# GATB/dsk

Measured on AMD Instinct MI355X. Metric: distinct k-mers counted/sec (whole node), k=31, higher is better.
Workload: dtype u64

## Files before the change

dsk_amd/csrc/dskgpu.hip:

```cpp
#include <algorithm>
#include <cstdio>
#include <cstring>
#include <cstdlib>
#include <cmath>
#include <string>
#include <vector>

#include <thread>
#include <system_error>
#include "engine.h"
#include "kernels.h"
#include "superkmer_recv.h"
#include "rawparse.h"

#include <rocprim/device/device_radix_sort.hpp>

#define DSKGPU_VERSION "dskgpu 0.1 (gfx950)"

namespace {

thread_local std::string g_create_err;

__global__ __launch_bounds__(1024) void k_place_probe(unsigned long long* __restrict__ out, unsigned long long n) {
    const unsigned long long per_block = n / gridDim.x, per_stream = per_block / 512;
// ... 115 lines not shown
    if ((reinterpret_cast<uintptr_t>(d_bytes) & 15) == 0)
        hipLaunchKernelGGL(k_encode<true>, dim3(grid), dim3(256), 0, ctx->stream, d_bytes, n, packed, inval, nwords);
    else
        hipLaunchKernelGGL(k_encode<false>, dim3(grid), dim3(256), 0, ctx->stream, d_bytes, n, packed, inval, nwords);
    CKL("k_encode");
    return DSKGPU_OK;
}

int run_scan(dskgpu_ctx* ctx, u32* a, const u32* d_len, u64 max_len) {
    const u64 nb = std::max<u64>(1, (max_len + SCAN_BLK - 1) / SCAN_BLK);
    CK(ctx->sums.ensure((nb + 1) * 4));
    hipLaunchKernelGGL(k_scan_reduce, dim3((unsigned)nb), dim3(SCAN_NT), 0, ctx->stream, a, d_len, ctx->sums.as<u32>());
    hipLaunchKernelGGL(k_scan_sums, dim3(1), dim3(1024), 0, ctx->stream, ctx->sums.as<u32>(), d_len, a);
    hipLaunchKernelGGL(k_scan_apply, dim3((unsigned)nb), dim3(SCAN_NT), 0, ctx->stream, a, d_len, ctx->sums.as<u32>());
    CKL("k_scan");
    return DSKGPU_OK;
}

int allow_big_lds(dskgpu_ctx* ctx, const void* fn, int bytes) {
    for (const void* f : ctx->big_lds_fns) if (f == fn) return DSKGPU_OK;
    CK(hipFuncSetAttribute(fn, hipFuncAttributeMaxDynamicSharedMemorySize, bytes));
    ctx->big_lds_fns.push_back(fn);
    return DSKGPU_OK;
}

namespace {

size_t scatter_lds(int W, u32 P, bool opt = false) { return (size_t)SC_NT * (16 / W) * 8 * W + (size_t)P * (opt ? 20 : 16) + 4 + 17 * 4 + 16 + (opt ? 8 + L0_MAX_PASSES * 8 : 0); }

template <int W, int SRC, int MODE>
int launch_hist_m(dskgpu_ctx* ctx, const typename KeyT<W>::T* keys, const ChunkDesc* descs, const u32* d_nch,
                  u64 max_chunks, u32* matrix, DigitSpec ds, u32 P) {
    const unsigned grid = (unsigned)std::max<u64>(1, std::min<u64>(max_chunks, (u64)ctx->num_cu));
    hipLaunchKernelGGL((k_hist<W, SRC, MODE>), dim3(grid), dim3(SC_NT), 0, ctx->stream, ctx->packed.as<u64>(),
                       ctx->inval.as<u32>(), keys, descs, d_nch, matrix, (int)ctx->cfg.kmer_size, ds, P);
    CKL("k_hist");
    return DSKGPU_OK;
}
template <int W, int SRC>
int launch_hist(dskgpu_ctx* ctx, const typename KeyT<W>::T* keys, const ChunkDesc* descs, const u32* d_nch,
                u64 max_chunks, u32* matrix, DigitSpec ds, u32 P) {
    const bool mp = ds.mode == 1 && ds.npass > 1;
    if (SRC == 0) return ds.mode == 0 ? launch_hist_m<W, 0, 0>(ctx, keys, descs, d_nch, max_chunks, matrix, ds, P)
                       : mp ? launch_hist_m<W, 0, 3>(ctx, keys, descs, d_nch, max_chunks, matrix, ds, P)
                            : launch_hist_m<W, 0, 1>(ctx, keys, descs, d_nch, max_chunks, matrix, ds, P);
    return ds.mode == 2 ? launch_hist_m<W, 1, 2>(ctx, keys, descs, d_nch, max_chunks, matrix, ds, P)
                   : mp ? launch_hist_m<W, 1, 3>(ctx, keys, descs, d_nch, max_chunks, matrix, ds, P)
                        : launch_hist_m<W, 1, 1>(ctx, keys, descs, d_nch, max_chunks, matrix, ds, P);
}

unsigned scatter_grid(const dskgpu_ctx* ctx, int W, u32 P, u64 max_chunks, bool opt = false) {
    const size_t lds = scatter_lds(W, P, opt);
    const u64 per_cu = std::max<u64>(1, std::min<u64>(2048 / SC_NT, (160 * 1024) / lds));
    return (unsigned)std::max<u64>(1, std::min<u64>(max_chunks, (u64)ctx->num_cu * per_cu));
}
template <int W, int SRC, int MODE, bool OPT = false, bool HEAVY = false>
int launch_scatter_m(dskgpu_ctx* ctx, const typename KeyT<W>::T* keys, const ChunkDesc* descs, const u32* d_nch,
                     u64 max_chunks, const u32* scanned, typename KeyT<W>::T* out, DigitSpec ds, u32 P, Opt1Spec o1 = Opt1Spec{nullptr, 0u, 0u, nullptr, nullptr, 0u, nullptr, nullptr, nullptr, 0u, nullptr, 0ull, {0ull, 0ull, 0ull, 0ull}, 0u}) {
    const size_t lds = scatter_lds(W, P, OPT && !o1.uslice);
    const unsigned grid = scatter_grid(ctx, W, P, max_chunks, OPT && !o1.uslice);
    { const int e = allow_big_lds(ctx, reinterpret_cast<const void*>(&k_scatter<W, SRC, MODE, OPT, HEAVY>)); if (e) return e; }
    hipLaunchKernelGGL((k_scatter<W, SRC, MODE, OPT, HEAVY>), dim3(grid), dim3(SC_NT), lds, ctx->stream, SRC == 2 ? ctx->rec_src : ctx->packed.as<u64>(),
                       SRC == 2 ? nullptr : ctx->inval.as<u32>(), keys, descs, d_nch, scanned, out, (int)ctx->cfg.kmer_size, ds, P, o1);
    CKL("k_scatter");
    return DSKGPU_OK;
}
template <int W, int MODE, bool OPT = false, bool SLICED = false>
int launch_scatter_al(dskgpu_ctx* ctx, const typename KeyT<W>::T* keys, const ChunkDesc* descs, const u32* d_nch,
                      u64 max_chunks, const u32* scanned, typename KeyT<W>::T* out, DigitSpec ds, u32 P, OptSpec os = OptSpec{0u, nullptr, nullptr, nullptr, 0u, 0u, 0ull, 0u, 0u, nullptr, nullptr, nullptr, nullptr, nullptr, nullptr}) {
    const size_t lds = ascatter_lds(W, P);
    const unsigned grid = (unsigned)std::max<u64>(1, std::min<u64>(max_chunks, (u64)ctx->num_cu));
    { const int e = allow_big_lds(ctx, reinterpret_cast<const void*>(&k_scatter_al<W, MODE, OPT, SLICED>)); if (e) return e; }
    hipLaunchKernelGGL((k_scatter_al<W, MODE, OPT, SLICED>), dim3(grid), dim3(SC_NT), lds, ctx->stream, keys, descs, d_nch, scanned, out, ds, P, os);
    CKL("k_scatter_al");
    return DSKGPU_OK;
}

template <int W, int SRC>
int launch_scatter(dskgpu_ctx* ctx, const typename KeyT<W>::T* keys, const ChunkDesc* descs, const u32* d_nch,
                   u64 max_chunks, const u32* scanned, typename KeyT<W>::T* out, DigitSpec ds, u32 P) {
    const bool mp = ds.mode == 1 && ds.npass > 1;
    if (SRC == 1 && ascatter_lds(W, P) <= 160 * 1024 && !ctx->tune.no_aligned)
        return ds.mode == 2 ? launch_scatter_al<W, 2>(ctx, keys, descs, d_nch, max_chunks, scanned, out, ds, P)
                       : mp ? launch_scatter_al<W, 3>(ctx, keys, descs, d_nch, max_chunks, scanned, out, ds, P)
                            : launch_scatter_al<W, 1>(ctx, keys, descs, d_nch, max_chunks, scanned, out, ds, P);
    if (SRC == 0) return ds.mode == 0 ? launch_scatter_m<W, 0, 0>(ctx, keys, descs, d_nch, max_chunks, scanned, out, ds, P)
                       : mp ? launch_scatter_m<W, 0, 3>(ctx, keys, descs, d_nch, max_chunks, scanned, out, ds, P)
                            : launch_scatter_m<W, 0, 1>(ctx, keys, descs, d_nch, max_chunks, scanned, out, ds, P);
    return ds.mode == 2 ? launch_scatter_m<W, 1, 2>(ctx, keys, descs, d_nch, max_chunks, scanned, out, ds, P)
                   : mp ? launch_scatter_m<W, 1, 3>(ctx, keys, descs, d_nch, max_chunks, scanned, out, ds, P)
                        : launch_scatter_m<W, 1, 1>(ctx, keys, descs, d_nch, max_chunks, scanned, out, ds, P);
}

inline void launch_count_impl(dskgpu_ctx* ctx, unsigned grid, u64* keys, u64* solid_keys, u32* solid_ab, u32* ovf, const CountParams& cp) {
    if (cp.cap && cp.cap <= CNT_V3_KEYS * CNT_NT) {
        hipLaunchKernelGGL((k_count1v3<CNT_NT, CNT_KPT, CNT_V3_KEYS>), dim3(grid), dim3(CNT_NT), 0, ctx->stream, keys, solid_keys, solid_ab,
                           ctx->nsolid.as<u32>(), ctx->ghist.as<u64>(), ctx->gstats.as<u64>(), ovf, cp, cp.subcnt);
        return;
    }
    if (cp.cap) hipLaunchKernelGGL(k_count1<true>, dim3(grid), dim3(CNT_NT), 0, ctx->stream, keys, solid_keys, ctx->fstart.as<u32>(), solid_ab,
                                   ctx->nsolid.as<u32>(), ctx->ghist.as<u64>(), ctx->gstats.as<u64>(), ovf, cp, cp.subcnt);
    else hipLaunchKernelGGL(k_count1<false>, dim3(grid), dim3(CNT_NT), 0, ctx->stream, keys, solid_keys, ctx->fstart.as<u32>(), solid_ab,
                            ctx->nsolid.as<u32>(), ctx->ghist.as<u64>(), ctx->gstats.as<u64>(), ovf, cp, (const u32*)ctx->fstart.as<u32>());
}
template <int W>
inline void launch_count_impl(dskgpu_ctx* ctx, unsigned grid, KN<W>* keys, KN<W>* solid_keys, u32* solid_ab, u32* ovf, const CountParams& cp) {
    if constexpr (W == 2) {
// ... 549 lines not shown
    ctx->mark("scatter1");
    return DSKGPU_OK;
}

template <int W>
int pass_scatter2(dskgpu_ctx* ctx, PassState<W>& ps) {
    const Plan& pl = ps.pl;
    int rc;
    ps.fkeys = ctx->bufA.as<typename KeyT<W>::T>();
    ps.scratch = &ctx->bufB;
    CK(ctx->fstart.ensure(((size_t)pl.F + 2) * 4));
    CK(ctx->nsolid.ensure(((size_t)pl.F + 2) * 4));
    if (pl.levels == 2 && ps.opt_cap) {
        CK(ctx->bufB.ensure((ps.nregions * ps.opt_cap + ATile<W>::KEYS + 16) * sizeof(typename KeyT<W>::T)));
        CK(ctx->descs2.ensure(((size_t)pl.P1 * 2 + 1) * sizeof(ChunkDesc)));
        CK(ctx->seg.ensure((size_t)pl.P1 * sizeof(SegInfo)));
        CK(ctx->mat2.ensure(((size_t)ps.nregions + 1) * 4));
        CK(ctx->chain_next.ensure(((size_t)ps.nregions + 1 + ps.max_ext + 1) * 4));
        if (ps.opt1) {
            ctx->h_descs2.resize(pl.P1);
            std::vector<u32> order(pl.P1);
            for (u32 sgm = 0; sgm < pl.P1; ++sgm) order[sgm] = sgm;
            double mean_work = 0.0; for (double w : ps.load) mean_work += w; mean_work = std::max(1.0, mean_work / pl.P1);
            auto wclass = [&](u32 a) { return (long long)(ps.load[a] / (0.05 * mean_work)); };
            std::stable_sort(order.begin(), order.end(), [&](u32 a, u32 b) { return wclass(a) > wclass(b); });
            for (u32 i = 0; i < pl.P1; ++i) {
                const u32 sgm = order[i];
                ChunkDesc d; d.begin = ctx->h_boff[sgm]; d.end = ctx->h_boff[sgm + 1]; d.flat_base = sgm * pl.P2; d.stride = 1;
                ctx->h_descs2[i] = d;
            }
            CK(hipMemcpyAsync(ctx->descs2.p, ctx->h_descs2.data(), (size_t)pl.P1 * sizeof(ChunkDesc), hipMemcpyHostToDevice, ctx->stream));
        } else {
            hipLaunchKernelGGL(k_plan, dim3(1), dim3(1024), 0, ctx->stream, ctx->mat1.as<u32>(), ps.nch1, pl.P1, 0x7FFFFFFFu, pl.P2,
                               ctx->seg.as<SegInfo>(), ctx->descs2.as<ChunkDesc>(), ps.sc + SC_NCH2, ps.sc + SC_MLEN2, 1u);
            CKL("k_plan");
        }
        ctx->mark("plan2");
        OptSpec os{ps.opt_cap, ctx->mat2.as<u32>(), ps.sc + SC_OVF2, ps.opt1 ? ps.o1.fill : nullptr, 0u, ps.grid1, (u64)ps.o1.area,
                   pl.F, ps.max_ext, ctx->chain_next.as<u32>(), ps.sc + SC_EXT, ctx->chain_next.as<u32>() + ps.nregions + 1, ps.sc + SC_NCHAINED,
                   ps.sc + SC_WORK2, nullptr};
        if (ctx->tune.verbose && ps.opt1) { CK(ctx->dbg.ensure((size_t)pl.P1 * 24)); os.dbg = ctx->dbg.as<unsigned long long>(); }
        if (ps.opt1) rc = launch_scatter_al<W, 2, true, true>(ctx, ctx->bufA.as<typename KeyT<W>::T>(), ctx->descs2.as<ChunkDesc>(), ps.sc + SC_NCH2, (u64)pl.P1 * 2, nullptr,
                                                              ctx->bufB.as<typename KeyT<W>::T>(), pl.d2, pl.P2, os);
        else rc = launch_scatter_al<W, 2, true, false>(ctx, ctx->bufA.as<typename KeyT<W>::T>(), ctx->descs2.as<ChunkDesc>(), ps.sc + SC_NCH2, (u64)pl.P1 * 2, nullptr,
                                                       ctx->bufB.as<typename KeyT<W>::T>(), pl.d2, pl.P2, os);
        if (rc) return rc;
        ctx->mark("scatter2");
        if (ctx->tune.verbose && ps.opt1) {
            std::vector<unsigned long long> t((size_t)pl.P1 * 3);
            CK(hipMemcpyAsync(t.data(), ctx->dbg.p, t.size() * 8, hipMemcpyDeviceToHost, ctx->stream));
            CK(hipStreamSynchronize(ctx->stream));
            unsigned long long t0 = ~0ull, t1 = 0; for (u32 i = 0; i < pl.P1; ++i) { t0 = std::min(t0, t[3 * i]); t1 = std::max(t1, t[3 * i + 1]); }
            fprintf(stderr, "[dskgpu] level 2: %u segments, %.3f ms first start -> last end\n", pl.P1, (t1 - t0) * 1e-5);
            for (u32 i = 0; i < pl.P1; ++i)
                if (i < 6 || i + 3 >= pl.P1 || t[3 * i + 1] + 20000 > t1)
                    fprintf(stderr, "[dskgpu]   desc %u (segment %u, load %.0f) block %llu: %.3f .. %.3f ms\n", i, (u32)(ctx->h_descs2[i].flat_base / pl.P2),
                            ps.load[ctx->h_descs2[i].flat_base / pl.P2], t[3 * i + 2], (t[3 * i] - t0) * 1e-5, (t[3 * i + 1] - t0) * 1e-5);
        }
        ps.fkeys = ctx->bufB.as<typename KeyT<W>::T>();
        ps.scratch = &ctx->bufA;
    } else if (pl.levels == 2) {
        const u64 max_chunks2 = ps.cap / CH2 + pl.P1 + 1;
        const u64 M2 = max_chunks2 * pl.P2;
        if (M2 >= 0xFFFFFFFFull) return fail(ctx, DSKGPU_E_ARG, "level-2 matrix too large");
        CK(ctx->descs2.ensure(max_chunks2 * sizeof(ChunkDesc)));
        CK(ctx->seg.ensure((size_t)pl.P1 * sizeof(SegInfo)));
        CK(ctx->mat2.ensure((M2 + 1) * 4));
        hipLaunchKernelGGL(k_plan, dim3(1), dim3(1024), 0, ctx->stream, ctx->mat1.as<u32>(), ps.nch1, pl.P1, CH2, pl.P2,
                           ctx->seg.as<SegInfo>(), ctx->descs2.as<ChunkDesc>(), ps.sc + SC_NCH2, ps.sc + SC_MLEN2, 0u);
        CKL("k_plan");
        ctx->mark("plan2");
        const ChunkDesc* dd2 = ctx->descs2.as<ChunkDesc>();
        if ((rc = launch_hist<W, 1>(ctx, ctx->bufA.as<typename KeyT<W>::T>(), dd2, ps.sc + SC_NCH2, max_chunks2, ctx->mat2.as<u32>(), pl.d2, pl.P2))) return rc;
        ctx->mark("hist2");
        if ((rc = run_scan(ctx, ctx->mat2.as<u32>(), ps.sc + SC_MLEN2, M2))) return rc;
        ctx->mark("scan2");
        if ((rc = launch_scatter<W, 1>(ctx, ctx->bufA.as<typename KeyT<W>::T>(), dd2, ps.sc + SC_NCH2, max_chunks2, ctx->mat2.as<u32>(), ctx->bufB.as<typename KeyT<W>::T>(), pl.d2, pl.P2))) return rc;
        ctx->mark("scatter2");
        ps.fkeys = ctx->bufB.as<typename KeyT<W>::T>();
        ps.scratch = &ctx->bufA;
        hipLaunchKernelGGL(k_final_offsets, dim3((pl.F + 256) / 256), dim3(256), 0, ctx->stream, ctx->mat2.as<u32>(),
                           ctx->seg.as<SegInfo>(), pl.P2, 0u, ps.sc + SC_MLEN2, ctx->fstart.as<u32>(), pl.F);
    } else {
        hipLaunchKernelGGL(k_final_offsets, dim3((pl.F + 256) / 256), dim3(256), 0, ctx->stream, ctx->mat1.as<u32>(),
                           (const SegInfo*)nullptr, pl.P1, ps.nch1, ps.sc + SC_MLEN1, ctx->fstart.as<u32>(), pl.F);
    }
    CKL("k_final_offsets");
    ctx->mark("offsets");
    return DSKGPU_OK;
}

template <int W>
int count_and_sizes(dskgpu_ctx* ctx, PassState<W>& ps, const CountParams& cp) {
    typedef typename KeyT<W>::T Key;
    const Plan& pl = ps.pl;
    const unsigned cgrid = (unsigned)std::min<u64>(pl.F, (u64)ctx->num_cu * 2);
    launch_count<W>(ctx, cgrid, ps.fkeys, ps.solid_keys, ps.solid_ab, ps.sc + SC_OVERFLOW, cp);
    CKL("k_count");
    if constexpr (W <= 2) {
        if (ps.opt_cap && ps.max_ext) {
            auto kern = [] { if constexpr (W == 1) return k_count_chained; else return k_count_chained_mw<2>; }();
            hipLaunchKernelGGL(kern, dim3((unsigned)std::min<u64>(ps.max_ext, (u64)ctx->num_cu * 2)), dim3(CNT_NT), 0, ctx->stream, ps.fkeys, ps.solid_keys, ps.solid_ab,
                               ctx->nsolid.as<u32>(), ctx->ghist.as<u64>(), ctx->gstats.as<u64>(), ps.sc + SC_OVERFLOW, cp, (const u32*)cp.subcnt,
                               (const u32*)ctx->chain_next.as<u32>(), (const u32*)(ctx->chain_next.as<u32>() + ps.nregions + 1), (const u32*)(ps.sc + SC_NCHAINED), ps.max_ext);
            CKL(W == 1 ? "k_count_chained" : "k_count_chained_mw");
        }
        if (ps.nheavy) {
            const u32 slots = HV_KEYS;
            u64* hvb = ctx->hv_buf.as<u64>();
            hipLaunchKernelGGL(k_heavy_rows<W>, dim3((slots + 255) / 256), dim3(256), 0, ctx->stream, reinterpret_cast<const Key*>(hvb + HvLayout<W>::keys),
// ... 1227 lines not shown
```

dsk_amd/csrc/engine.h:

```cpp
#pragma once
#include <algorithm>
#include <cstring>
#include <string>
#include <vector>

#include "../../include/dskgpu.h"
#include "layouts.h"

hipError_t placed_malloc(void** out, size_t bytes);

struct DevBuf {
    void* p = nullptr;
    size_t cap = 0;
    hipError_t ensure(size_t bytes) {
        if (bytes <= cap) return hipSuccess;
        size_t want = ((p ? bytes + bytes / 16 : bytes) + 255) & ~size_t(255);
        if (p) { (void)hipFree(p); p = nullptr; cap = 0; }
        hipError_t e = placed_malloc(&p, want);
        if (e == hipSuccess) cap = want; else p = nullptr;
        return e;
    }
    int ensure_keep(size_t bytes, size_t keep, hipStream_t stream) {
        if (bytes <= cap) return 0;
        void* np = nullptr;
        size_t want = ((std::max(bytes, cap + cap / 2) + 255) & ~size_t(255));
        if (hipMalloc(&np, want) != hipSuccess) return -1;
        if (keep && p) {
            if (hipMemcpyAsync(np, p, keep, hipMemcpyDeviceToDevice, stream) != hipSuccess || hipStreamSynchronize(stream) != hipSuccess) { (void)hipFree(np); return -1; }
        }
        if (p) (void)hipFree(p);
        p = np; cap = want;
        return 0;
    }
    void release() { if (p) (void)hipFree(p); p = nullptr; cap = 0; }
    template <class T> T* as() const { return reinterpret_cast<T*>(p); }
};

enum Scalar { SC_NCH1 = 0, SC_MLEN1, SC_NCH2, SC_MLEN2, SC_OVERFLOW, SC_F, SC_SORTFLAG, SC_OVF2, SC_OVF1, SC_RSLEN, SC_RSWORK, SC_RSWORK2, SC_RSTIES, SC_EXT, SC_NCHAINED, SC_NCH_S, SC_MLEN_S, SC_WORK2, SC_COUNT = 24 };

struct Stage { const char* name; hipEvent_t ev; };

struct Tuning {
    bool no_opt1 = false, no_opt2 = false;
    bool no_aligned = false;
    u32 rs_heavy = 0;
    u32 rs_bbits = 0;
    u32 rs_block_rows = 0;
    bool sk_exact = false, no_recsrc = false;
    u32 opt_cap = 0;
    u64 opt_slice = 0;
    u64 sk_slice = 0, sk_minslice = 2000;
    u32 table_maxload = 0;
    long long max_ext = -1;
    bool no_sample = false;
    bool no_heavy = false;
    bool verbose = false;
    bool no_level0 = false; u32 l0_passes = 0;
    u64 rs_max_rows = 0;
    u32 ps_maxc = 0;
    bool sk_generic = false;
    bool l0_keys = false;
    u32 mp_pass_mkeys = 0;
    u64 rs_slab_rows = 0;
    bool unitig_stages = false;
    bool cc_plain = false, cc_stages = false;
    bool correct_staged = false;
    u32 pairs_reg_max = ~0u, pairs_grid = 0; bool pairs_no_skip = false;
    void read() {
        auto on =[](const char* n) { return getenv(n) != nullptr; };
        auto num = [](const char* n, u64 dflt) { const char* e = getenv(n); return e ? (u64)atoll(e) : dflt; };
        no_opt1 = on("DSKGPU_NO_OPT1"); no_opt2 = on("DSKGPU_NO_OPT2"); no_aligned = on("DSKGPU_NO_ALIGNED");
        sk_exact = on("DSKGPU_SK_EXACT");
        no_recsrc = on("DSKGPU_NO_RECSRC");
        opt_cap = (u32)num("DSKGPU_OPT_CAP", 0) & ~7u; opt_slice = num("DSKGPU_OPT_SLICE", 0) & ~7ull;
        sk_slice = num("DSKGPU_SK_SLICE", 0); sk_minslice = num("DSKGPU_SK_MINSLICE", 2000);
        table_maxload = (u32)num("DSKGPU_TABLE_MAXLOAD", 0);
        max_ext = getenv("DSKGPU_MAX_EXT") ? atoll(getenv("DSKGPU_MAX_EXT")) : -1;
        no_sample = on("DSKGPU_NO_SAMPLE"); no_heavy = on("DSKGPU_NO_HEAVY"); verbose = on("DSKGPU_VERBOSE"); no_level0 = on("DSKGPU_NO_LEVEL0"); l0_passes = (u32)num("DSKGPU_L0_PASSES", 0); mp_pass_mkeys = (u32)num("DSKGPU_MP_PASS_MKEYS", 0); rs_max_rows = num("DSKGPU_RS_MAX_ROWS", 0); l0_keys = on("DSKGPU_L0_KEYS"); sk_generic = on("DSKGPU_SK_GENERIC"); ps_maxc = (u32)num("DSKGPU_PS_MAXC", 0);
        rs_slab_rows = num("DSKGPU_RS_SLAB_ROWS", 0);
        unitig_stages = on("DSKGPU_UNITIG_STAGES");
        cc_plain = on("DSKGPU_CC_PLAIN"); cc_stages = on("DSKGPU_CC_STAGES");
        correct_staged = on("DSKGPU_CORRECT_STAGED");
        pairs_reg_max = (u32)num("DSKGPU_PAIRS_REG_MAX", pairs_reg_max); pairs_no_skip = on("DSKGPU_PAIRS_NO_SKIP"); pairs_grid = (u32)num("DSKGPU_PAIRS_GRID", 0);
        rs_block_rows = (u32)num("DSKGPU_RS_BLOCK_ROWS", 0); rs_bbits = (u32)num("DSKGPU_RS_BBITS", 0); rs_heavy = (u32)num("DSKGPU_RS_HEAVY", 0);
    }
};

struct SparseRows {
    int W = 0;
    const void* keys = nullptr; const u32 *ab = nullptr, *soff = nullptr, *fstart = nullptr; u32 cap = 0, F = 0;
    u64 n_sparse = 0; u32 n_tail = 0; RowsIn tail_w{}; const u32* tail_ab = nullptr;
    template <class S> S as(u32 qpc = 0) const { return S{static_cast<decltype(S::keys)>(keys), ab, soff, fstart, cap, F, qpc}; }
    Rows2C tail2() const { return Rows2C{tail_w.w[1], tail_w.w[0], tail_ab}; }
};

struct PartPasses {
    struct Pass { u64 row_base; u32 nparts, off_index; };
    std::vector<Pass> passes; DevBuf part_off, flag; u32 off_used = 0; bool ok = false; u64 row_base = 0;
    std::vector<u32> h_off;
};

struct RowSort {
    DevBuf fix_list;
    DevBuf g[4];
    DevBuf del, lens;
    std::vector<u64> h_del; std::vector<u32> h_lens, h_lin;
    DevBuf ovs;
    u32 flag = 0, listed = 0;
    u64* hist_pin = nullptr; size_t hist_pin_n = 0;
    bool part_mode = false; u32 n_parts = 0; u32* h_part_off = nullptr; size_t h_part_cap = 0; DevBuf part_off;
    std::vector<u64> h_part_off64;
    PartPasses mp;
    void release() {
        for (DevBuf* b : {&fix_list, &g[0], &g[1], &g[2], &g[3], &del, &lens, &ovs, &part_off, &mp.part_off, &mp.flag}) b->release();
        if (hist_pin) (void)hipHostFree(hist_pin);
        if (h_part_off) (void)hipHostFree(h_part_off);
        hist_pin = nullptr; h_part_off = nullptr;
    }
};

struct Query {
    DevBuf table, packed, inval, deg;
    u64 cap = 0;
    bool valid = false;
    void release() { table.release(); packed.release(); inval.release(); deg.release(); cap = 0; valid = false; }
    void invalidate() { valid = false; }
};

struct Components {
    DevBuf comp, first, cols;
    dskgpu_component_stats stats{};
    bool valid = false;
// ... 248 lines not shown
```

dsk_amd/csrc/kernels.h:

```cpp
#pragma once
#include "layouts.h"

#ifndef SC_NT
#define SC_NT 1024
#endif
template <int W> struct Tile {
    static constexpr int KPT = 16 / W;
    static constexpr int KEYS = SC_NT * KPT;
    static constexpr int WORDS = KEYS / 32;
};
#define MAX_BINS 2048


template <bool ALIGNED>
__global__ __launch_bounds__(256) void k_encode(const uint8_t* __restrict__ s, u64 n,
                                                u64* __restrict__ packed, u32* __restrict__ inval, u64 nwords) {
    const u64 stride = (u64)gridDim.x * blockDim.x;
    for (u64 w = (u64)blockIdx.x * blockDim.x + threadIdx.x; w < nwords; w += stride) {
        const u64 base = w * 32;
        u32 x[8];
        if (ALIGNED && base + 32 <= n) {
            const uint4 a = *reinterpret_cast<const uint4*>(s + base);
            const uint4 b = *reinterpret_cast<const uint4*>(s + base + 16);
            x[0] = a.x; x[1] = a.y; x[2] = a.z; x[3] = a.w; x[4] = b.x; x[5] = b.y; x[6] = b.z; x[7] = b.w;
// ... 717 lines not shown
            }
            const int f = ic ? __clz((int)ic) : 32;
            const int need = k - 1 - run;
            const int good = f - (need > 0 ? need : 0);
            c += good > 0 ? (u32)good : 0u;
        }
    }
#pragma unroll
    for (int d = 32; d >= 1; d >>= 1) c += __shfl_down(c, d);
    if ((threadIdx.x & 63) == 0) ws[threadIdx.x >> 6] = c;
    __syncthreads();
    if (threadIdx.x == 0) atomicAdd(total, (u64)ws[0] + ws[1] + ws[2] + ws[3]);
}

#ifndef AL_G2
#define AL_G2 4
#define AL_KPT2 6
#endif
#ifndef AL_G1
#define AL_G1 8
#define AL_KPT1 12
#endif
template <int W> struct ATile {
    static constexpr int G = W == 2 ? AL_G2 : W == 1 ? AL_G1 : 8 / W;
    static constexpr int CARRY = G - 1;
    static constexpr int KPT = W == 2 ? AL_KPT2 : W == 1 ? AL_KPT1 : 12 / W;
    static constexpr int KEYS = SC_NT * KPT;
};
#define AL_BIG 64
#define AL_BIG_KEYS 64u
#ifndef SLICED_MAX
#define SLICED_MAX 320
#endif
__host__ __device__ inline size_t ascatter_lds(int W, u32 P) {
    const size_t key = 8 * (size_t)W, keys = (size_t)SC_NT * (W == 2 ? AL_KPT2 : W == 1 ? AL_KPT1 : 12 / W), G = W == 2 ? AL_G2 : W == 1 ? AL_G1 : 8 / W;
    return keys * key + (size_t)P * (G - 1) * key + (size_t)(P + 1) * 4 + (size_t)P * 4 + (size_t)(P + 1) * 12 + (size_t)P * 2 + 20 * 4 + 32
           + SLICED_MAX * 4 + 16
           + 2 * AL_BIG * 2 + 16;
}

template <int W, int MODE, bool OPT = false, bool SLICED = false>
__global__ __launch_bounds__(SC_NT, 4) void k_scatter_al(const typename KeyT<W>::T* __restrict__ keys,
                                                         const ChunkDesc* __restrict__ descs, const u32* __restrict__ d_nchunks,
                                                         const u32* __restrict__ scanned,
                                                         typename KeyT<W>::T* __restrict__ out_all, DigitSpec ds, u32 P, OptSpec os) {
    typedef typename KeyT<W>::T Key;
    typedef unsigned short u16;
    constexpr int KPT = ATile<W>::KPT, G = ATile<W>::G, CARRY = ATile<W>::CARRY, TKEYS = ATile<W>::KEYS;
    constexpr int NGRP = SC_NT / G;
    extern __shared__ __attribute__((aligned(16))) char smem[];
    Key* stage = reinterpret_cast<Key*>(smem);
    Key* carry = stage + TKEYS;
    u32* cnt = reinterpret_cast<u32*>(carry + (size_t)P * CARRY);
    u32* pos = cnt + (P + 1);
    uint3* rec = reinterpret_cast<uint3*>(pos + P);
    u16* rn = reinterpret_cast<u16*>(rec + (P + 1));
    u32* wsum = reinterpret_cast<u32*>(smem + ((reinterpret_cast<char*>(rn + P) - smem + 3) & ~size_t(3)));
    u32* pre = wsum + 20;
    u16* big = reinterpret_cast<u16*>(pre + SLICED_MAX + 4);
    const int tid = threadIdx.x, lane = tid & 63, wave = tid >> 6;
    const u32 gi = tid / G, gl = tid % G;
    const u32 nchunks = *d_nchunks;
    const int ipt = (int)((P + SC_NT - 1) / SC_NT);
    u32 g = blockIdx.x;
    for (;; ) {
        if (g >= nchunks) break;
        const ChunkDesc d = descs[g];
        if (OPT && os.dbg && tid == 0) { os.dbg[3 * g] = wall_clock64(); os.dbg[3 * g + 2] = blockIdx.x; }
        Key* out = OPT ? out_all + (u64)d.flat_base * os.cap : out_all;
        Key* extb = OPT ? out_all + (u64)os.F * os.cap : out_all;
        bool ovf = false;
        lds_barrier();
        for (u32 b = tid; b < P; b += SC_NT) { pos[b] = OPT ? b * os.cap : scanned[d.flat_base + (u64)b * d.stride]; cnt[b] = 0; rn[b] = 0; }
        if (tid == 0) { cnt[P] = 0; wsum[17] = 0; wsum[18] = 0; }
        u32 par = 0;
        u64 lbeg = d.begin, lend = d.end;
        u32 sg = 0, slo = 0, shi = 0;
        if (SLICED) {
            if (wave == 0) {
                const u32* f = os.fill + (u64)(d.flat_base / P) * os.nsl;
                u32 run = 0;
                for (u32 i0 = 0; i0 < os.nsl; i0 += 64) {
                    const u32 i = i0 + lane;
                    const u32 v = i < os.nsl ? f[i] : 0u;
                    u32 inc = v;
#pragma unroll
                    for (int dd = 1; dd < 64; dd <<= 1) { const u32 t = __shfl_up(inc, dd); if (lane >= dd) inc += t; }
                    if (i < os.nsl) pre[i] = run + inc - v;
                    run += __shfl(inc, 63);
                }
                if (lane == 0) pre[os.nsl] = run;
            }
            lds_barrier();
            lbeg = 0; lend = pre[os.nsl];
            shi = pre[1];
        }
        Key h[KPT]; u32 vm = 0;
        auto load = [&](u64 k0, Key (&hh)[KPT]) -> u32 {
            const Key* base = keys + (SLICED ? d.begin : k0);
            const u64 left = lend - k0;
            const u32 n = left < (u64)TKEYS ? (u32)left : (u32)TKEYS;
            u32 m = 0;
#pragma unroll
            for (int j = 0; j < KPT; ++j) {
                const u32 o = tid + (u32)j * SC_NT;
                const bool ok = o < n;
                if (!SLICED) hh[j] = base[ok ? o : n - 1];
                else {
                    const u32 i = (u32)k0 + (ok ? o : n - 1);
                    while (i >= shi && sg + 1 < os.nsl) { ++sg; slo = shi; shi = pre[sg + 1]; }
                    const u32 off = i >= slo ? i - slo : 0u;
                    hh[j] = base[(u64)sg * os.sstride + off];
                }
                m |= (ok ? 1u : 0u) << j;
            }
            return m;
        };
        auto process = [&](u64 tnext) {
            u32 rk[KPT];
#pragma unroll
            for (int j = 0; j < KPT; ++j) {
                const bool pad = (OPT && is_empty_key(h[j])) || is_pad_key(h[j]);
                u32 dj = key_digit<MODE>(digit_word(h[j]), ds);
                asm volatile("" : "+v"(dj));
                dj = ((vm & (1u << j)) && !pad && key_in_pass<MODE>(digit_word(h[j]), ds)) ? dj : P;
                rk[j] = dj << 16;
            }
#pragma unroll
            for (int j = 0; j < KPT; ++j) rk[j] |= atomicAdd(&cnt[rk[j] >> 16], 1u);
            lds_barrier();
            if (tid == 0) {
                cnt[P] = 0;
                wsum[17 + (par ^ 1u)] = 0;
            }
            {
                const int base = tid * ipt;
                u32 c[4], pe[4], er[4], s = 0;
#pragma unroll
                for (int j = 0; j < 4; ++j) {
                    const int b = base + j;
                    c[j] = 0; pe[j] = 0; er[j] = 0;
                    if (j < ipt && b < (int)P) {
                        c[j] = cnt[b];
                        const u32 r = rn[b]; u32 p = pos[b];
                        const u32 pl = OPT ? p & ~CHAIN_BIT : p;
                        const u32 bound = (pl + r + c[j]) & ~(u32)(G - 1);
                        const u32 e = bound > pl ? bound - pl : 0u;
                        if (OPT) {
                            const bool ext = (p >> 31) != 0u;
                            const u32 rs = ext ? pl / os.cap * os.cap : (u32)b * os.cap;
                            if (pl + e >= rs + os.cap) {
                                const u32 need = e / os.cap + 1u;
                                const u32 x = atomicAdd(os.ext_cursor, need);
                                if (x + need > os.max_ext) { ovf = true; p = (u32)b * os.cap; }
                                else {
                                    const u32 cur = ext ? os.F + pl / os.cap : d.flat_base + (u32)b;
                                    os.subcnt[cur] = CHAIN_BIT | (pl - rs); os.next[cur] = os.F + x;
                                    if (!ext) os.chain_list[atomicAdd(os.chain_cnt, 1u)] = cur;
                                    for (u32 i = 0; i + 1 < need; ++i) { os.subcnt[os.F + x + i] = CHAIN_BIT | os.cap; os.next[os.F + x + i] = os.F + x + i + 1u; }
                                    p = CHAIN_BIT | (x * os.cap);
                                }
                            }
                        }
                        pe[j] = p; er[j] = e | (r << 16);
                        rn[b] = (u16)(r + c[j] - e);
                        pos[b] = p + e; cnt[b] = 0;
                        if (e > AL_BIG_KEYS) { const u32 x = atomicAdd(&wsum[17 + par], 1u); if (x < AL_BIG) big[par * AL_BIG + x] = (u16)b; else er[j] |= 0x8000u; }
                    }
                    s += c[j];
                }
                const u32 inc = wave_incl_scan(s);
                if (lane == 63) wsum[wave] = inc;
                lds_barrier();
                if (wave == 0) {
                    const u32 x = lane < SC_NT / 64 ? wsum[lane] : 0u;
                    const u32 y = wave_incl_scan(x);
                    if (lane < SC_NT / 64) wsum[lane] = y - x;
                    if (lane == SC_NT / 64 - 1) rec[P].z = y;
                }
                lds_barrier();
                u32 run = wsum[wave] + inc - s;
#pragma unroll
                for (int j = 0; j < 4; ++j) {
                    const int b = base + j;
                    if (j < ipt && b < (int)P) { rec[b] = make_uint3(pe[j], er[j], run); run += c[j]; }
                }
            }
            lds_barrier();
            {
                u32 so[KPT];
#pragma unroll
                for (int j = 0; j < KPT; ++j) so[j] = rec[rk[j] >> 16].z;
#pragma unroll
                for (int j = 0; j < KPT; ++j) stage[so[j] + (rk[j] & 0xFFFFu)] = h[j];
            }
            if (tnext < lend) vm = load(tnext, h);
            lds_barrier();
            {
                const u32 nb = wsum[17 + par] < (u32)AL_BIG ? wsum[17 + par] : (u32)AL_BIG;
                for (u32 x = 0; x < nb; ++x) {
                    const uint3 rbig = rec[big[par * AL_BIG + x]];
                    const u32 e = rbig.y & 0x7FFFu, r = rbig.y >> 16, o = rbig.z;
                    const u32 pl = OPT ? rbig.x & ~CHAIN_BIT : rbig.x;
                    Key* ob = (OPT && (rbig.x >> 31)) ? extb : out;
                    for (u32 idx = G + tid; idx < e; idx += SC_NT) ob[pl + idx] = stage[o + idx - r];
                }
            }
            for (u32 b0 = 0; b0 < P; b0 += 2 * NGRP) {
                uint3 rb[2]; u32 rnew[2]; bool act[2];
#pragma unroll
                for (int u = 0; u < 2; ++u) {
                    const u32 b = b0 + u * NGRP + gi;
                    act[u] = b < P;
                    rb[u] = rec[act[u] ? b : 0]; rnew[u] = rn[act[u] ? b : 0];
                }
#pragma unroll
                for (int u = 0; u < 2; ++u) {
                    if (!act[u]) continue;
                    const u32 b = b0 + u * NGRP + gi;
                    const u32 e = rb[u].y & 0x7FFFu, r = rb[u].y >> 16, o = rb[u].z;
                    const u32 mine = (e > AL_BIG_KEYS && !(rb[u].y & 0x8000u)) ? (u32)G : e;
                    const u32 pold = OPT ? rb[u].x & ~CHAIN_BIT : rb[u].x;
                    Key* ob = (OPT && (rb[u].x >> 31)) ? extb : out;
                    Key* cb = carry + (size_t)b * CARRY;
                    for (u32 a = (pold & ~(u32)(G - 1)) + gl; a < pold + mine; a += G) {
                        if (a >= pold) {
                            const u32 idx = a - pold;
                            const Key kv = idx < r ? cb[idx] : stage[o + idx - r];
                            ob[a] = kv;
                        }
                    }
                    const u32 c = rnew[u] + e - r;
                    if (e) { if (gl < rnew[u]) cb[gl] = stage[o + c - rnew[u] + gl]; }
                    else if (gl < c) cb[r + gl] = stage[o + gl];
                }
            }
            par ^= 1u;
        };
        if (lbeg < lend) vm = load(lbeg, h);
        lds_barrier();
        for (u64 t0 = lbeg; t0 < lend; t0 += (u64)TKEYS) process(t0 + TKEYS);
        lds_barrier();
        for (u32 b = gi; b < P; b += NGRP) {
            const u32 r = rn[b];
            if (!OPT) { if (gl < r) out[pos[b] + gl] = carry[(size_t)b * CARRY + gl]; }
            else {
                const u32 p = pos[b], pl = p & ~CHAIN_BIT;
                const bool ext = (p >> 31) != 0u;
                const u32 rs = ext ? pl / os.cap * os.cap : b * os.cap;
                Key* ob = ext ? extb : out;
                if (r) ob[pl + gl] = gl < r ? carry[(size_t)b * CARRY + gl] : empty_key<W>();
                if (gl == 0) os.subcnt[ext ? os.F + pl / os.cap : d.flat_base + b] = pl - rs + r;
            }
        }
        if (OPT && ovf) *os.ovf = 1u;
        if (OPT && os.dbg && tid == 0) os.dbg[3 * g + 1] = wall_clock64();
        if (OPT && os.work) {
            lds_barrier();
            if (tid == 0) wsum[19] = atomicAdd(os.work, 1u);
            lds_barrier();
            g = wsum[19];
        } else g += gridDim.x;
    }
}

struct SegInfo { u32 start, nch, chunk_base, pad; };

__global__ __launch_bounds__(1024) void k_plan(const u32* __restrict__ src, u32 sstride, u32 S, u32 CH, u32 P,
                                               SegInfo* __restrict__ seg, ChunkDesc* __restrict__ descs,
                                               u32* __restrict__ d_nchunks, u32* __restrict__ d_mlen, u32 opt) {
    __shared__ u32 ws[16]; __shared__ u32 carry_s;
    const int lane = threadIdx.x & 63, wave = threadIdx.x >> 6;
    if (threadIdx.x == 0) carry_s = 0;
    __syncthreads();
    for (u32 s0 = 0; s0 < S; s0 += 1024) {
        const u32 s = s0 + threadIdx.x;
        u32 start = 0, size = 0, nch = 0;
        if (s < S) { start = src[(u64)s * sstride]; size = src[(u64)(s + 1) * sstride] - start; nch = (size + CH - 1) / CH; }
        u32 y = nch;
#pragma unroll
        for (int d = 1; d < 64; d <<= 1) { const u32 t = __shfl_up(y, d); if (lane >= d) y += t; }
        if (lane == 63) ws[wave] = y;
        __syncthreads();
        if (wave == 0) {
            const u32 wx = lane < 16 ? ws[lane] : 0u; u32 wy = wx;
#pragma unroll
            for (int d = 1; d < 16; d <<= 1) { const u32 t = __shfl_up(wy, d); if (lane >= d) wy += t; }
            if (lane < 16) ws[lane] = wy - wx;
        }
        __syncthreads();
        const u32 cb = carry_s + ws[wave] + y - nch;
        if (s < S) {
            SegInfo si; si.start = start; si.nch = nch; si.chunk_base = cb; si.pad = 0;
            seg[s] = si;
            for (u32 c = 0; c < nch; ++c) {
                ChunkDesc d;
                d.begin = (u64)start + (u64)c * CH;
                const u64 e = d.begin + CH, lim = (u64)start + size;
                d.end = e < lim ? e : lim;
                d.flat_base = opt ? s * P : cb * P + c;
                d.stride = nch;
                descs[cb + c] = d;
            }
        }
        __syncthreads();
        if (threadIdx.x == 1023) carry_s = cb + nch;
        __syncthreads();
    }
    if (threadIdx.x == 0) { *d_nchunks = carry_s; *d_mlen = carry_s * P; }
// ... 1091 lines not shown
```

Measured before the change: 26.89 billion.

## Add full-tile fast path and split scatter bucket records in sliced scatter

In the sliced level-2 scatter kernel, tiles that are wave-uniformly full (narrow keys) skip the per-key pad, empty and pass checks when computing digits. The per-bucket LDS record shrinks from uint3 to uint2, with the stage offset moved to its own array so the key-placement gather reads a single u32. Bucket bookkeeping is factored into a lambda with a dedicated one-bucket-per-thread path, and thread-index copies are pinned in VGPRs via asm barriers. It also adds a DSKGPU_L1_GRID env cap on the level-1 scatter grid and verbose loader tile statistics. The fast path assumes full tiles of width 2 or less never contain pad keys.

```diff
diff --git a/dsk_amd/csrc/dskgpu.hip b/dsk_amd/csrc/dskgpu.hip
--- a/dsk_amd/csrc/dskgpu.hip
+++ b/dsk_amd/csrc/dskgpu.hip
@@ -191,7 +191,9 @@
 unsigned scatter_grid(const dskgpu_ctx* ctx, int W, u32 P, u64 max_chunks, bool opt = false) {
     const size_t lds = scatter_lds(W, P, opt);
     const u64 per_cu = std::max<u64>(1, std::min<u64>(2048 / SC_NT, (160 * 1024) / lds));
-    return (unsigned)std::max<u64>(1, std::min<u64>(max_chunks, (u64)ctx->num_cu * per_cu));
+    u64 grid = std::min<u64>(max_chunks, (u64)ctx->num_cu * per_cu);
+    if (ctx->tune.l1_grid) grid = std::min<u64>(grid, ctx->tune.l1_grid);
+    return (unsigned)std::max<u64>(1, grid);
 }
 template <int W, int SRC, int MODE, bool OPT = false, bool HEAVY = false>
 int launch_scatter_m(dskgpu_ctx* ctx, const typename KeyT<W>::T* keys, const ChunkDesc* descs, const u32* d_nch,
@@ -847,10 +849,17 @@
             CK(hipStreamSynchronize(ctx->stream));
             unsigned long long t0 = ~0ull, t1 = 0; for (u32 i = 0; i < pl.P1; ++i) { t0 = std::min(t0, t[3 * i]); t1 = std::max(t1, t[3 * i + 1]); }
             fprintf(stderr, "[dskgpu] level 2: %u segments, %.3f ms first start -> last end\n", pl.P1, (t1 - t0) * 1e-5);
+            unsigned long long nfull = 0, npart = 0; u32 nseg_full = 0, nseg_part = 0, nseg_empty = 0;
+            for (u32 i = 0; i < pl.P1; ++i) {
+                const unsigned long long f = (t[3 * i + 2] >> 16) & 0xFFFFFFull, w = t[3 * i + 2] >> 40;
+                nfull += f; npart += w; nseg_full += f != 0; nseg_part += w != 0; nseg_empty += (f | w) == 0;
+            }
+            fprintf(stderr, "[dskgpu] level 2 loader: %llu full tiles in %u segments, %llu clamped tiles in %u segments, %u empty segments, %u slices per segment\n",
+                    nfull, nseg_full, npart, nseg_part, nseg_empty, ps.grid1);
             for (u32 i = 0; i < pl.P1; ++i)
                 if (i < 6 || i + 3 >= pl.P1 || t[3 * i + 1] + 20000 > t1)
                     fprintf(stderr, "[dskgpu]   desc %u (segment %u, load %.0f) block %llu: %.3f .. %.3f ms\n", i, (u32)(ctx->h_descs2[i].flat_base / pl.P2),
-                            ps.load[ctx->h_descs2[i].flat_base / pl.P2], t[3 * i + 2], (t[3 * i] - t0) * 1e-5, (t[3 * i + 1] - t0) * 1e-5);
+                            ps.load[ctx->h_descs2[i].flat_base / pl.P2], t[3 * i + 2] & 0xFFFFull, (t[3 * i] - t0) * 1e-5, (t[3 * i + 1] - t0) * 1e-5);
         }
         ps.fkeys = ctx->bufB.as<typename KeyT<W>::T>();
         ps.scratch = &ctx->bufA;
diff --git a/dsk_amd/csrc/engine.h b/dsk_amd/csrc/engine.h
--- a/dsk_amd/csrc/engine.h
+++ b/dsk_amd/csrc/engine.h
@@ -49,6 +49,7 @@
     bool sk_exact = false, no_recsrc = false;
     u32 opt_cap = 0;
     u64 opt_slice = 0;
+    u32 l1_grid = 0;
     u64 sk_slice = 0, sk_minslice = 2000;
     u32 table_maxload = 0;
     long long max_ext = -1;
@@ -78,6 +79,7 @@
         max_ext = getenv("DSKGPU_MAX_EXT") ? atoll(getenv("DSKGPU_MAX_EXT")) : -1;
         no_sample = on("DSKGPU_NO_SAMPLE"); no_heavy = on("DSKGPU_NO_HEAVY"); verbose = on("DSKGPU_VERBOSE"); no_level0 = on("DSKGPU_NO_LEVEL0"); l0_passes = (u32)num("DSKGPU_L0_PASSES", 0); mp_pass_mkeys = (u32)num("DSKGPU_MP_PASS_MKEYS", 0); rs_max_rows = num("DSKGPU_RS_MAX_ROWS", 0); l0_keys = on("DSKGPU_L0_KEYS"); sk_generic = on("DSKGPU_SK_GENERIC"); ps_maxc = (u32)num("DSKGPU_PS_MAXC", 0);
         rs_slab_rows = num("DSKGPU_RS_SLAB_ROWS", 0);
+        l1_grid = (u32)num("DSKGPU_L1_GRID", 0);
         unitig_stages = on("DSKGPU_UNITIG_STAGES");
         cc_plain = on("DSKGPU_CC_PLAIN"); cc_stages = on("DSKGPU_CC_STAGES");
         correct_staged = on("DSKGPU_CORRECT_STAGED");
diff --git a/dsk_amd/csrc/kernels.h b/dsk_amd/csrc/kernels.h
--- a/dsk_amd/csrc/kernels.h
+++ b/dsk_amd/csrc/kernels.h
@@ -793,9 +793,10 @@
     Key* stage = reinterpret_cast<Key*>(smem);
     Key* carry = stage + TKEYS;
     u32* cnt = reinterpret_cast<u32*>(carry + (size_t)P * CARRY);
-    u32* pos = cnt + (P + 1);
-    uint3* rec = reinterpret_cast<uint3*>(pos + P);
-    u16* rn = reinterpret_cast<u16*>(rec + (P + 1));
+    u32* soff = cnt + (P + 1);
+    uint2* rec = reinterpret_cast<uint2*>(soff + (P + 1));
+    u32* pos = reinterpret_cast<u32*>(rec + P);
+    u16* rn = reinterpret_cast<u16*>(pos + P);
     u32* wsum = reinterpret_cast<u32*>(smem + ((reinterpret_cast<char*>(rn + P) - smem + 3) & ~size_t(3)));
     u32* pre = wsum + 20;
     u16* big = reinterpret_cast<u16*>(pre + SLICED_MAX + 4);
@@ -807,22 +808,23 @@
     for (;; ) {
         if (g >= nchunks) break;
         const ChunkDesc d = descs[g];
-        if (OPT && os.dbg && tid == 0) { os.dbg[3 * g] = wall_clock64(); os.dbg[3 * g + 2] = blockIdx.x; }
+        if (OPT && os.dbg && tid == 0) os.dbg[3 * g] = wall_clock64();
         Key* out = OPT ? out_all + (u64)d.flat_base * os.cap : out_all;
         Key* extb = OPT ? out_all + (u64)os.F * os.cap : out_all;
         bool ovf = false;
+        u32 ts = (u32)tid;
+        asm volatile("" : "+v"(ts));
         lds_barrier();
-        for (u32 b = tid; b < P; b += SC_NT) { pos[b] = OPT ? b * os.cap : scanned[d.flat_base + (u64)b * d.stride]; cnt[b] = 0; rn[b] = 0; }
+        for (u32 b = ts; b < P; b += SC_NT) { pos[b] = OPT ? b * os.cap : scanned[d.flat_base + (u64)b * d.stride]; cnt[b] = 0; rn[b] = 0; }
         if (tid == 0) { cnt[P] = 0; wsum[17] = 0; wsum[18] = 0; }
         u32 par = 0;
         u64 lbeg = d.begin, lend = d.end;
-        u32 sg = 0, slo = 0, shi = 0;
         if (SLICED) {
             if (wave == 0) {
                 const u32* f = os.fill + (u64)(d.flat_base / P) * os.nsl;
                 u32 run = 0;
                 for (u32 i0 = 0; i0 < os.nsl; i0 += 64) {
-                    const u32 i = i0 + lane;
+                    const u32 i = i0 + (ts & 63u);
                     const u32 v = i < os.nsl ? f[i] : 0u;
                     u32 inc = v;
 #pragma unroll
@@ -834,17 +836,26 @@
             }
             lds_barrier();
             lbeg = 0; lend = pre[os.nsl];
-            shi = pre[1];
-        }
+        }
+        u32 sg = 0, slo = 0, shi = 0;
+        if (SLICED) shi = pre[1];
+        u32 nfull = 0, npart = 0;
         Key h[KPT]; u32 vm = 0;
-        auto load = [&](u64 k0, Key (&hh)[KPT]) -> u32 {
+        bool hfull = false;
+        auto load = [&](u64 k0, Key (&hh)[KPT]) __attribute__((always_inline)) -> u32 {
             const Key* base = keys + (SLICED ? d.begin : k0);
             const u64 left = lend - k0;
             const u32 n = left < (u64)TKEYS ? (u32)left : (u32)TKEYS;
+            u32 tq = (u32)tid;
+            asm volatile("" : "+v"(tq));
+            if constexpr (SLICED) {
+                hfull = W <= 2 && __builtin_amdgcn_readfirstlane(n) == (u32)TKEYS;
+                if (n == (u32)TKEYS) ++nfull; else ++npart;
+            }
             u32 m = 0;
 #pragma unroll
             for (int j = 0; j < KPT; ++j) {
-                const u32 o = tid + (u32)j * SC_NT;
+                const u32 o = tq + (u32)j * SC_NT;
                 const bool ok = o < n;
                 if (!SLICED) hh[j] = base[ok ? o : n - 1];
                 else {
@@ -859,13 +870,18 @@
         };
         auto process = [&](u64 tnext) {
             u32 rk[KPT];
-#pragma unroll
-            for (int j = 0; j < KPT; ++j) {
-                const bool pad = (OPT && is_empty_key(h[j])) || is_pad_key(h[j]);
-                u32 dj = key_digit<MODE>(digit_word(h[j]), ds);
-                asm volatile("" : "+v"(dj));
-                dj = ((vm & (1u << j)) && !pad && key_in_pass<MODE>(digit_word(h[j]), ds)) ? dj : P;
-                rk[j] = dj << 16;
+            if (SLICED && hfull) {
+#pragma unroll
+                for (int j = 0; j < KPT; ++j) rk[j] = key_digit<MODE>(digit_word(h[j]), ds) << 16;
+            } else {
+#pragma unroll
+                for (int j = 0; j < KPT; ++j) {
+                    const bool pad = (!SLICED || W > 2) && ((OPT && is_empty_key(h[j])) || is_pad_key(h[j]));
+                    u32 dj = key_digit<MODE>(digit_word(h[j]), ds);
+                    asm volatile("" : "+v"(dj));
+                    dj = ((vm & (1u << j)) && !pad && key_in_pass<MODE>(digit_word(h[j]), ds)) ? dj : P;
+                    rk[j] = dj << 16;
+                }
             }
 #pragma unroll
             for (int j = 0; j < KPT; ++j) rk[j] |= atomicAdd(&cnt[rk[j] >> 16], 1u);
@@ -875,40 +891,43 @@
                 wsum[17 + (par ^ 1u)] = 0;
             }
             {
-                const int base = tid * ipt;
-                u32 c[4], pe[4], er[4], s = 0;
-#pragma unroll
-                for (int j = 0; j < 4; ++j) {
-                    const int b = base + j;
-                    c[j] = 0; pe[j] = 0; er[j] = 0;
-                    if (j < ipt && b < (int)P) {
-                        c[j] = cnt[b];
-                        const u32 r = rn[b]; u32 p = pos[b];
-                        const u32 pl = OPT ? p & ~CHAIN_BIT : p;
-                        const u32 bound = (pl + r + c[j]) & ~(u32)(G - 1);
-                        const u32 e = bound > pl ? bound - pl : 0u;
-                        if (OPT) {
-                            const bool ext = (p >> 31) != 0u;
-                            const u32 rs = ext ? pl / os.cap * os.cap : (u32)b * os.cap;
-                            if (pl + e >= rs + os.cap) {
-                                const u32 need = e / os.cap + 1u;
-                                const u32 x = atomicAdd(os.ext_cursor, need);
-                                if (x + need > os.max_ext) { ovf = true; p = (u32)b * os.cap; }
-                                else {
-                                    const u32 cur = ext ? os.F + pl / os.cap : d.flat_base + (u32)b;
-                                    os.subcnt[cur] = CHAIN_BIT | (pl - rs); os.next[cur] = os.F + x;
-                                    if (!ext) os.chain_list[atomicAdd(os.chain_cnt, 1u)] = cur;
-                                    for (u32 i = 0; i + 1 < need; ++i) { os.subcnt[os.F + x + i] = CHAIN_BIT | os.cap; os.next[os.F + x + i] = os.F + x + i + 1u; }
-                                    p = CHAIN_BIT | (x * os.cap);
-                                }
+                auto book = [&](const u32 b, u32& c, u32& pe, u32& er) {
+                    c = cnt[b];
+                    const u32 r = rn[b]; u32 p = pos[b];
+                    const u32 pl = OPT ? p & ~CHAIN_BIT : p;
+                    const u32 bound = (pl + r + c) & ~(u32)(G - 1);
+                    const u32 e = bound > pl ? bound - pl : 0u;
+                    if (OPT) {
+                        const bool ext = (p >> 31) != 0u;
+                        const u32 rs = ext ? pl / os.cap * os.cap : b * os.cap;
+                        if (pl + e >= rs + os.cap) {
+                            const u32 need = e / os.cap + 1u;
+                            const u32 x = atomicAdd(os.ext_cursor, need);
+                            if (x + need > os.max_ext) { ovf = true; p = b * os.cap; }
+                            else {
+                                const u32 cur = ext ? os.F + pl / os.cap : d.flat_base + b;
+                                os.subcnt[cur] = CHAIN_BIT | (pl - rs); os.next[cur] = os.F + x;
+                                if (!ext) os.chain_list[atomicAdd(os.chain_cnt, 1u)] = cur;
+                                for (u32 i = 0; i + 1 < need; ++i) { os.subcnt[os.F + x + i] = CHAIN_BIT | os.cap; os.next[os.F + x + i] = os.F + x + i + 1u; }
+                                p = CHAIN_BIT | (x * os.cap);
                             }
                         }
-                        pe[j] = p; er[j] = e | (r << 16);
-                        rn[b] = (u16)(r + c[j] - e);
-                        pos[b] = p + e; cnt[b] = 0;
-                        if (e > AL_BIG_KEYS) { const u32 x = atomicAdd(&wsum[17 + par], 1u); if (x < AL_BIG) big[par * AL_BIG + x] = (u16)b; else er[j] |= 0x8000u; }
                     }
-                    s += c[j];
+                    pe = p; er = e | (r << 16);
+                    rn[b] = (u16)(r + c - e);
+                    pos[b] = p + e; cnt[b] = 0;
+                    if (e > AL_BIG_KEYS) { const u32 x = atomicAdd(&wsum[17 + par], 1u); if (x < AL_BIG) big[par * AL_BIG + x] = (u16)b; else er |= 0x8000u; }
+                };
+                const int base = tid * ipt;
+                u32 c[4] = {0u, 0u, 0u, 0u}, pe[4] = {0u, 0u, 0u, 0u}, er[4] = {0u, 0u, 0u, 0u}, s = 0;
+                if (ipt == 1) { if (tid < (int)P) book((u32)tid, c[0], pe[0], er[0]); s = c[0]; }
+                else {
+#pragma unroll
+                    for (int j = 0; j < 4; ++j) {
+                        const int b = base + j;
+                        if (j < ipt && b < (int)P) book((u32)b, c[j], pe[j], er[j]);
+                        s += c[j];
+                    }
                 }
                 const u32 inc = wave_incl_scan(s);
                 if (lane == 63) wsum[wave] = inc;
@@ -917,21 +936,24 @@
                     const u32 x = lane < SC_NT / 64 ? wsum[lane] : 0u;
                     const u32 y = wave_incl_scan(x);
                     if (lane < SC_NT / 64) wsum[lane] = y - x;
-                    if (lane == SC_NT / 64 - 1) rec[P].z = y;
+                    if (lane == SC_NT / 64 - 1) soff[P] = y;
                 }
                 lds_barrier();
                 u32 run = wsum[wave] + inc - s;
-#pragma unroll
-                for (int j = 0; j < 4; ++j) {
-                    const int b = base + j;
-                    if (j < ipt && b < (int)P) { rec[b] = make_uint3(pe[j], er[j], run); run += c[j]; }
+                if (ipt == 1) { if (tid < (int)P) { rec[tid] = make_uint2(pe[0], er[0]); soff[tid] = run; } }
+                else {
+#pragma unroll
+                    for (int j = 0; j < 4; ++j) {
+                        const int b = base + j;
+                        if (j < ipt && b < (int)P) { rec[b] = make_uint2(pe[j], er[j]); soff[b] = run; run += c[j]; }
+                    }
                 }
             }
             lds_barrier();
             {
                 u32 so[KPT];
 #pragma unroll
-                for (int j = 0; j < KPT; ++j) so[j] = rec[rk[j] >> 16].z;
+                for (int j = 0; j < KPT; ++j) so[j] = soff[rk[j] >> 16];
 #pragma unroll
                 for (int j = 0; j < KPT; ++j) stage[so[j] + (rk[j] & 0xFFFFu)] = h[j];
             }
@@ -940,26 +962,27 @@
             {
                 const u32 nb = wsum[17 + par] < (u32)AL_BIG ? wsum[17 + par] : (u32)AL_BIG;
                 for (u32 x = 0; x < nb; ++x) {
-                    const uint3 rbig = rec[big[par * AL_BIG + x]];
-                    const u32 e = rbig.y & 0x7FFFu, r = rbig.y >> 16, o = rbig.z;
+                    const u32 bb = big[par * AL_BIG + x];
+                    const uint2 rbig = rec[bb];
+                    const u32 e = rbig.y & 0x7FFFu, r = rbig.y >> 16, o = soff[bb];
                     const u32 pl = OPT ? rbig.x & ~CHAIN_BIT : rbig.x;
                     Key* ob = (OPT && (rbig.x >> 31)) ? extb : out;
                     for (u32 idx = G + tid; idx < e; idx += SC_NT) ob[pl + idx] = stage[o + idx - r];
                 }
             }
             for (u32 b0 = 0; b0 < P; b0 += 2 * NGRP) {
-                uint3 rb[2]; u32 rnew[2]; bool act[2];
+                uint2 rb[2]; u32 ob2[2], rnew[2]; bool act[2];
 #pragma unroll
                 for (int u = 0; u < 2; ++u) {
                     const u32 b = b0 + u * NGRP + gi;
                     act[u] = b < P;
-                    rb[u] = rec[act[u] ? b : 0]; rnew[u] = rn[act[u] ? b : 0];
+                    rb[u] = rec[act[u] ? b : 0]; ob2[u] = soff[act[u] ? b : 0]; rnew[u] = rn[act[u] ? b : 0];
                 }
 #pragma unroll
                 for (int u = 0; u < 2; ++u) {
                     if (!act[u]) continue;
                     const u32 b = b0 + u * NGRP + gi;
-                    const u32 e = rb[u].y & 0x7FFFu, r = rb[u].y >> 16, o = rb[u].z;
+                    const u32 e = rb[u].y & 0x7FFFu, r = rb[u].y >> 16, o = ob2[u];
                     const u32 mine = (e > AL_BIG_KEYS && !(rb[u].y & 0x8000u)) ? (u32)G : e;
                     const u32 pold = OPT ? rb[u].x & ~CHAIN_BIT : rb[u].x;
                     Key* ob = (OPT && (rb[u].x >> 31)) ? extb : out;
@@ -982,7 +1005,9 @@
         lds_barrier();
         for (u64 t0 = lbeg; t0 < lend; t0 += (u64)TKEYS) process(t0 + TKEYS);
         lds_barrier();
-        for (u32 b = gi; b < P; b += NGRP) {
+        asm volatile("" : "+v"(ts));
+        for (u32 b = ts / G; b < P; b += NGRP) {
+            const u32 gl = ts % G;
             const u32 r = rn[b];
             if (!OPT) { if (gl < r) out[pos[b] + gl] = carry[(size_t)b * CARRY + gl]; }
             else {
@@ -996,6 +1021,7 @@
         }
         if (OPT && ovf) *os.ovf = 1u;
         if (OPT && os.dbg && tid == 0) os.dbg[3 * g + 1] = wall_clock64();
+        if (OPT && os.dbg && tid == SC_NT - 64) os.dbg[3 * g + 2] = (u64)blockIdx.x | ((u64)nfull << 16) | ((u64)npart << 40);
         if (OPT && os.work) {
             lds_barrier();
             if (tid == 0) wsum[19] = atomicAdd(os.work, 1u);
```

Result: no change. 26.74 billion (-0.6%).
